# al8n/serf

Measured on NVIDIA H100. Metric: gossip edge-updates/sec @10M nodes, higher is better.
Workload: dtype u32

## Files before the change

### serf_b200/csrc/serfsim.cu

```cuda
#include <algorithm>
#include <cmath>
#include <cstdio>
#include <cstdlib>
#include <cstring>
#include <string>
#include <unordered_set>
#include <vector>

#include "../../include/serfsim.h"
#include "tick_kernel.cuh"
#include "wire.cuh"

using namespace sfs;

namespace {

thread_local std::string g_err;

int fail(int code, const std::string& msg) { g_err = msg; return code; }

#define CU(call)                                                                              \
  do {                                                                                        \
    cudaError_t e_ = (call);                                                                  \
    if (e_ != cudaSuccess)                                                                    \
// ... 50 lines not shown
    tab.push_back((u32)ticks);
  }
  return tab;
}

struct Switches {
  int gridmul = 2;
  bool minb5 = false;
  bool tma = false;
  bool tma_sync = false;
  bool udeg = true;
  u32 ahead = 1;
  u32 sv = 1;
  bool compact = true;
  bool dedup = true;
  bool no_skip = false;
  bool no_jump = false;
  u32 chunk = 0;
  double win_factor = 1.25;
  bool no_fuse = false;
  int l2_persist = 0;
  bool l2_window = false;
  bool verbose = false;
  bool debug_loop = false;
  bool xtiming = false;
};

Switches read_switches() {
  auto num = [](const char* name, int dflt) { const char* e = getenv(name); return e ? atoi(e) : dflt; };
  auto set = [](const char* name) { return getenv(name) != nullptr; };
  Switches s;
  s.gridmul = num("SERFSIM_GRIDMUL", s.gridmul); if (s.gridmul < 1) s.gridmul = 2;
  s.minb5 = num("SERFSIM_MINB", 0) == 5;
  s.tma = num("SERFSIM_TMA", s.tma) != 0;
  s.tma_sync = num("SERFSIM_TMA_SYNC", s.tma_sync) != 0;
  s.udeg = num("SERFSIM_UDEG", s.udeg) != 0;
  s.ahead = (u32)std::min(2, std::max(0, num("SERFSIM_AHEAD", s.ahead)));
  s.sv = (u32)std::min(2, std::max(0, num("SERFSIM_SV", s.sv)));
  s.compact = num("SERFSIM_COMPACT", s.compact) != 0;
  s.dedup = num("SERFSIM_DEDUP", s.dedup) != 0;
  s.no_skip = num("SERFSIM_NO_SKIP", s.no_skip) != 0;
  s.no_jump = set("SERFSIM_NO_JUMP");
  s.chunk = set("SERFSIM_CHUNK") ? (u32)std::max(1, num("SERFSIM_CHUNK", 1)) : 0u;
  if (const char* e = getenv("SERFSIM_WIN_FACTOR")) s.win_factor = atof(e);
  s.no_fuse = set("SERFSIM_NO_FUSE");
  s.l2_persist = num("SERFSIM_L2_PERSIST", s.l2_persist);
  s.l2_window = num("SERFSIM_L2_WINDOW", s.l2_window) != 0;
  s.verbose = set("SERFSIM_VERBOSE");
  s.debug_loop = set("SERFSIM_DEBUG_LOOP");
  s.xtiming = set("SERFSIM_XTIMING");
  return s;
}

}

// ... 15 lines not shown
  const u64** d_peer_snap_node = nullptr;
  u8* d_hot[2] = {nullptr, nullptr};
  u8* d_hot_static = nullptr;
  u32* d_node_due = nullptr;
  u32* d_carry = nullptr;
  u32* d_tile_due = nullptr;
  u32* d_sched = nullptr;
  u32 n_tiles = 0;
  u32* d_rowptr = nullptr;
  u32* d_col = nullptr;
  u32 *d_ev_node = nullptr, *d_ev_op = nullptr, *d_ev_slot = nullptr;
  size_t ev_cap = 0;
  u64* d_trace = nullptr;
  u32* d_kinds = nullptr;
  u32* d_view_kinds = nullptr;
  u32 trace_cap = 0;
  u32* d_overflow = nullptr;
  u32* pin_overflow = nullptr;
  u32* d_subj = nullptr;
  u64* d_scratch = nullptr;
  void* d_stage = nullptr;
  UeTable ue_table{};
  uint4* d_ue_state = nullptr;
  u32* d_ue_inbox[2] = {nullptr, nullptr};
  u32* d_ue_ltime = nullptr;
  wire::UeWire ue_wire{};
  u8* d_ue_entries = nullptr;
  u64* d_ue_totals = nullptr;
  u32 ue_injected = 0;
  uint4* d_ue_snap = nullptr;
// ... 62 lines not shown
  std::vector<cudaEvent_t> tick_ev;
  std::vector<cudaEvent_t> mid_ev;
};

namespace {

int slot_of(const serfsim* h, u32 node) {
  for (u32 s = 0; s < h->R; ++s) if (h->subj[s] == node) return (int)s;
  return -1;
}

int ensure_trace(serfsim* h, u32 need) {
  if (need <= h->trace_cap) return 0;
  u32 cap = std::max<u32>(1024, h->trace_cap);
  while (cap < need) cap *= 2;
  u64* nt = nullptr; u32* nk = nullptr; u32* nv = nullptr; u64* ng = nullptr;
  const bool sharded = h->cfg.world_size > 1;
  CU(cudaMalloc(&nt, (size_t)cap * 8 * sizeof(u64)));
  CU(cudaMalloc(&nk, ((size_t)cap + 1) * 4 * sizeof(u32)));
  CU(cudaMalloc(&nv, ((size_t)cap + 1) * h->R * 4 * sizeof(u32)));
  CU(cudaMemsetAsync(nt, 0, (size_t)cap * 8 * sizeof(u64), h->stream));
  CU(cudaMemsetAsync(nk, 0, ((size_t)cap + 1) * 4 * sizeof(u32), h->stream));
  CU(cudaMemsetAsync(nv, 0, ((size_t)cap + 1) * h->R * 4 * sizeof(u32), h->stream));
  if (sharded) { CU(cudaMalloc(&ng, (size_t)cap * 8 * sizeof(u64))); CU(cudaMemsetAsync(ng, 0, (size_t)cap * 8 * sizeof(u64), h->stream)); }
  if (h->d_trace) {
    CU(cudaMemcpyAsync(nt, h->d_trace, (size_t)h->trace_cap * 8 * sizeof(u64), cudaMemcpyDeviceToDevice, h->stream));
    CU(cudaMemcpyAsync(nk, h->d_kinds, ((size_t)h->trace_cap + 1) * 4 * sizeof(u32), cudaMemcpyDeviceToDevice, h->stream));
    CU(cudaMemcpyAsync(nv, h->d_view_kinds, ((size_t)h->trace_cap + 1) * h->R * 4 * sizeof(u32), cudaMemcpyDeviceToDevice, h->stream));
    if (sharded) CU(cudaMemcpyAsync(ng, h->d_grow, (size_t)h->trace_cap * 8 * sizeof(u64), cudaMemcpyDeviceToDevice, h->stream));
    CU(cudaStreamSynchronize(h->stream));
    cudaFree(h->d_trace); cudaFree(h->d_kinds); cudaFree(h->d_view_kinds); cudaFree(h->d_grow);
  }
  h->d_trace = nt; h->d_kinds = nk; h->d_view_kinds = nv; h->d_grow = ng; h->trace_cap = cap;
  return 0;
}

int upload_ops(serfsim* h) {
  if (!h->ops_dirty) return 0;
  std::stable_sort(h->ops.begin(), h->ops.end(), [](const HostOp& a, const HostOp& b) { return a.tick != b.tick ? a.tick < b.tick : a.seq < b.seq; });
  const size_t n = h->ops.size();
  if (n > h->ev_cap) {
    size_t cap = std::max<size_t>(1024, h->ev_cap);
    while (cap < n) cap *= 2;
    if (h->d_ev_node) { cudaFree(h->d_ev_node); cudaFree(h->d_ev_op); cudaFree(h->d_ev_slot); }
    CU(cudaMalloc(&h->d_ev_node, cap * 4)); CU(cudaMalloc(&h->d_ev_op, cap * 4)); CU(cudaMalloc(&h->d_ev_slot, cap * 4));
    h->ev_cap = cap;
  }
  if (n) {
// ... 32 lines not shown
    if (__builtin_popcount(h->ever_down) != 1) return TickRun::General;
    return h->sw.sv == 2 ? TickRun::Check : TickRun::Dual;
  }
  if (ops_at(h, t) || reap_tick(h, t) || t + 1 >= CARRY_TICKS) return TickRun::General;
  return h->sw.sv == 2 ? TickRun::Check : TickRun::Passes;
}
bool view_kinds_valid(const serfsim* h, u32 t) {
  return tick_run(h, t) == TickRun::Passes && !pp_tick(h, t);
}

TickParams at_view(const serfsim* h, const TickParams& p, u32 s) {
  TickParams q = p;
  q.sv_wshift = s;
  q.rec = p.rec + 2 * (size_t)s * h->stride; q.qword = p.qword + (size_t)s * h->stride;
  q.inbox_rd = p.inbox_rd + (size_t)s * h->stride; q.inbox_wr = p.inbox_wr + (size_t)s * h->stride;
  q.subj[0] = p.subj[s]; q.down_mask = (p.down_mask >> s) & 1u;
  q.tiles_per_cta = (h->n_tiles + h->grid_sv - 1) / h->grid_sv;
  return q;
}

int grow_events(std::vector<cudaEvent_t>& ev, size_t n) {
  while (ev.size() < n) { cudaEvent_t e; CU(cudaEventCreate(&e)); ev.push_back(e); }
  return 0;
}

int ue_cluster_ltimes(serfsim* h, u32 lt[MAX_UEVENTS]) {
  CU(cudaMemcpy(lt, h->d_ue_ltime, MAX_UEVENTS * sizeof(u32), cudaMemcpyDeviceToHost));
  if (h->cfg.world_size > 1 && h->allreduce) {
    u64 v[MAX_UEVENTS];
    for (u32 e = 0; e < MAX_UEVENTS; ++e) v[e] = (((h->ue_injected >> e) & 1u) && h->ue_origin[e] - h->first < h->count) ? lt[e] : 0;
// ... 26 lines not shown
  p.rec = h->d_rec; p.qword = h->d_qword; p.inbox_rd = h->d_inbox[(t & 1) ^ 1]; p.inbox_wr = h->d_inbox[t & 1];
  p.node_state = h->d_node; p.busy = h->d_busy; p.watch = h->d_watch; p.row_ptr = h->d_rowptr; p.col = h->d_col;
  p.ev_node = h->d_ev_node; p.ev_op = h->d_ev_op; p.ev_slot = h->d_ev_slot;
  p.row = h->d_trace + (size_t)t * 8;
  p.kinds_prev = h->d_kinds + (size_t)t * 4;
  p.kinds_cur = h->d_kinds + ((size_t)t + 1) * 4;
  p.overflow = h->d_overflow;
  p.hot_rd = h->d_hot[(t & 1) ^ 1]; p.hot_wr = h->d_hot[t & 1];
  p.stage_col_bytes = h->stage_col_bytes;
  p.reap_now = reap_tick(h, t) ? 1u : 0u;
  p.tombstone_ticks = h->cfg.tombstone_timeout_ticks; p.reconnect_ticks = h->cfg.reconnect_timeout_ticks; p.intent_ticks = h->cfg.recent_intent_timeout_ticks;
  p.stride = h->stride; p.n_tiles = h->n_tiles; p.tiles_per_cta = (h->n_tiles + h->grid - 1) / h->grid;
  p.force_all = (h->cfg.trace != 0) || h->sw.no_skip || p.reap_now;
  p.compact = h->sw.compact ? 1u : 0u;
  p.dedup = h->sw.dedup ? 1u : 0u;
  p.udeg = h->udeg; p.ahead = h->sw.ahead;
  p.tile_due = h->d_tile_due; p.node_due = h->d_node_due; p.hot_static = h->d_hot_static; p.sched = h->d_sched;
  p.sleep_on = (h->sw.no_skip || h->byz_on) ? 0u : 1u;
  p.pp_every = (u32)std::max(0, h->cfg.push_pull_interval_ticks); p.reap_every = h->cfg.reap_interval_ticks;
  p.host_idle_until = h->d_pin_ctl + 2;
  const bool sharded = h->cfg.world_size > 1;
  const u32 xpar = h->xepoch & 1;
  p.world = (u32)h->cfg.world_size; p.rank = (u32)h->cfg.rank; p.shard_size = h->shard_size; p.win_cap = h->win_cap;
  p.win_data = h->d_peer_data[xpar]; p.send_count = h->d_send_count;
  p.peer_ctrl = h->d_peer_ctrl; p.stamp = h->xepoch + 1; p.xpar = xpar; p.loopback = h->loopback ? 1u : 0u;
  p.fuse_publish = (sharded && !h->byz_on && !h->sw.no_fuse) ? 1u : 0u;
  p.shard_inv = (u32)(0x100000000ull / h->shard_size); p.xcap = p.world > 1 ? 392u / (p.world - 1) : 0u;
  if (h->gate_on) {
    const u64* grow = sharded ? h->d_grow : h->d_trace;
    Gate& g = p.gate;
// ... 251 lines not shown
  CU(cudaMemsetAsync(h->d_ue_ltime, 0, MAX_UEVENTS * 4, h->stream));
  CU(cudaMemsetAsync(h->d_ue_totals, 0, 8 * 8, h->stream));
  CU(cudaGetLastError());
  return 0;
}

int do_reset(serfsim* h, u64 seed) {
  h->cfg.seed = seed; h->tick = 0; h->ops.clear(); h->op_keys.clear(); h->ops_dirty = false; h->rows.clear();
  h->up_mask = (h->R >= 32) ? 0xffffffffu : ((1u << h->R) - 1);
  h->ever_down = 0;
  h->reported.assign(h->R, (u8)ST_ALIVE);
  const size_t inbox_bytes = (size_t)3 * h->R * h->stride * sizeof(u32);
  launch_init_state(h->d_rec, h->d_node, h->count, h->stride, h->R, h->cfg.init_status_ltime, h->cfg.init_clock, h->stream);
  CU(cudaMemsetAsync(h->d_inbox[0], 0, inbox_bytes, h->stream));
  CU(cudaMemsetAsync(h->d_inbox[1], 0, inbox_bytes, h->stream));
  CU(cudaStreamSynchronize(h->stream));
  *(volatile u32*)h->pin_overflow = 0;
  ((volatile u32*)h->pin_ctl)[2] = 0;
  CU(cudaMemsetAsync(h->d_busy, 0, h->stride, h->stream));
  CU(cudaMemsetAsync(h->d_qword, 0, (size_t)h->R * h->stride * 4, h->stream));
  CU(cudaMemsetAsync(h->d_hot[0], 0, h->n_tiles, h->stream));
  CU(cudaMemsetAsync(h->d_hot[1], 0, h->n_tiles, h->stream));
  CU(cudaMemsetAsync(h->d_tile_due, 0xff, (size_t)h->n_tiles * sizeof(u32), h->stream));
  CU(cudaMemsetAsync(h->d_node_due, 0xff, (size_t)h->stride * sizeof(u32), h->stream));
  if (h->d_carry) CU(cudaMemsetAsync(h->d_carry, 0, (size_t)h->stride * sizeof(u32), h->stream));
  CU(cudaMemsetAsync(h->d_sched, 0, SCHED_WORDS * sizeof(u32), h->stream));
  if (h->d_trace) {
    CU(cudaMemsetAsync(h->d_trace, 0, (size_t)h->trace_cap * 8 * sizeof(u64), h->stream));
    CU(cudaMemsetAsync(h->d_kinds, 0, ((size_t)h->trace_cap + 1) * 4 * sizeof(u32), h->stream));
    CU(cudaMemsetAsync(h->d_view_kinds, 0, ((size_t)h->trace_cap + 1) * h->R * 4 * sizeof(u32), h->stream));
  }
  if (h->d_grow) CU(cudaMemsetAsync(h->d_grow, 0, (size_t)h->trace_cap * 8 * sizeof(u64), h->stream));
  CU(cudaMemsetAsync(h->d_runctl, 0, 2 * sizeof(u32), h->stream));
  if (h->d_send_count) CU(cudaMemsetAsync(h->d_send_count, 0, sizeof(u32) * 8, h->stream));
  { int rc = ue_reset(h); if (rc) return rc; }
  if (h->d_anomaly) { CU(cudaMemsetAsync(h->d_anomaly, 0, h->stride, h->stream)); CU(cudaMemsetAsync(h->d_byz_totals, 0, 4 * 8, h->stream)); }
  { int rc = refresh_watchers(h); if (rc) return rc; }
  CU(cudaStreamSynchronize(h->stream));
  return 0;
}

void free_all(serfsim* h) {
  for (void* p : h->ipc_opened) cudaIpcCloseMemHandle(p);
  for (cudaEvent_t e : h->tick_ev) cudaEventDestroy(e);
  cudaFree(h->d_hot_static); cudaFree(h->d_tile_due); cudaFree(h->d_node_due); cudaFree(h->d_carry); cudaFree(h->d_sched);
  cudaFree(h->d_hot[0]); cudaFree(h->d_hot[1]); cudaFree(h->d_busy); cudaFree(h->d_watch); cudaFree(h->d_snap_rec); cudaFree(h->d_snap_node); cudaFree(h->d_peer_snap_rec); cudaFree(h->d_peer_snap_node);
  cudaFree(h->d_qword);
  cudaFree(h->d_rec); cudaFree(h->d_inbox[0]); cudaFree(h->d_inbox[1]); cudaFree(h->d_node); cudaFree(h->d_rowptr); cudaFree(h->d_col);
  cudaFree(h->d_ev_node); cudaFree(h->d_ev_op); cudaFree(h->d_ev_slot); cudaFree(h->d_trace); cudaFree(h->d_kinds); cudaFree(h->d_view_kinds);
  if (h->pin_overflow) cudaFreeHost(h->pin_overflow);
  cudaFree(h->d_subj); cudaFree(h->d_scratch); cudaFree(h->d_stage);
  cudaFree(h->d_byz_ids); cudaFree(h->d_anomaly); cudaFree(h->d_byz_totals); cudaFree(h->d_peer_anomaly);
  cudaFree(h->d_ue_snap); cudaFree(h->d_peer_ue_snap);
  cudaFree(h->d_ue_entries);
  cudaFree(h->d_ue_state); cudaFree(h->d_ue_inbox[0]); cudaFree(h->d_ue_inbox[1]); cudaFree(h->d_ue_ltime); cudaFree(h->d_ue_totals);
  for (int par = 0; par < 2; ++par) { cudaFree(h->d_win_data[par]); cudaFree(h->d_peer_data[par]); }
  cudaFree(h->d_ctrl); cudaFree(h->d_send_count); cudaFree(h->d_peer_ctrl);
  for (auto& b : h->res) { cudaFree(b.d); if (b.copied) cudaEventDestroy(b.copied); }
  if (h->ev_extracted) cudaEventDestroy(h->ev_extracted);
  if (h->copy_stream) cudaStreamDestroy(h->copy_stream);
  if (h->pin_ctl) cudaFreeHost(h->pin_ctl);
  cudaFree(h->d_runctl); cudaFree(h->d_grow);
  if (h->ev0) cudaEventDestroy(h->ev0);
  if (h->ev1) cudaEventDestroy(h->ev1);
// ... 121 lines not shown
  CUB(cudaMalloc(&h->d_hot_static, h->n_tiles)); CUB(cudaMalloc(&h->d_tile_due, (size_t)h->n_tiles * sizeof(u32))); CUB(cudaMalloc(&h->d_node_due, (size_t)h->stride * sizeof(u32))); CUB(cudaMalloc(&h->d_sched, SCHED_WORDS * sizeof(u32)));
  CUB(cudaMemset(h->d_hot_static, 0, h->n_tiles));
  if (h->R > 1 && cfg->world_size <= 1) CUB(cudaMalloc(&h->d_carry, (size_t)h->stride * sizeof(u32)));
  CUB(cudaHostAlloc(&h->pin_overflow, sizeof(u32), cudaHostAllocMapped));
  CUB(cudaHostGetDevicePointer(&h->d_overflow, h->pin_overflow, 0));
  *h->pin_overflow = 0;
  CUB(cudaMalloc(&h->d_subj, MAX_SLOTS * 4)); CUB(cudaMalloc(&h->d_scratch, 64 * 8));
  CUB(cudaMalloc(&h->d_stage, (size_t)h->count * 8));
  CUB(cudaMalloc(&h->d_runctl, 2 * sizeof(u32)));
  CUB(cudaMemset(h->d_runctl, 0, 2 * sizeof(u32)));
  CUB(cudaHostAlloc(&h->pin_ctl, 4 * sizeof(u32), cudaHostAllocMapped));
  CUB(cudaHostGetDevicePointer(&h->d_pin_ctl, h->pin_ctl, 0));
  h->pin_ctl[0] = h->pin_ctl[1] = h->pin_ctl[2] = h->pin_ctl[3] = 0;
  CUB(cudaMemcpy(h->d_subj, h->subj.data(), h->R * 4, cudaMemcpyHostToDevice));
  h->sw = read_switches();
  cudaDeviceGetAttribute(&h->sms, cudaDevAttrMultiProcessorCount, dev);
  if (h->sms <= 0) h->sms = 132;
  const int ctas_r1 = cfg->world_size > 1 ? tick_ctas_per_sm_r1s() : tick_ctas_per_sm_r1();
  h->ctas_per_sm = h->R > 1 ? tick_ctas_per_sm_rn() : h->sw.minb5 ? 5 : ctas_r1;
  h->grid = tick_grid_size(h->count, h->ctas_per_sm, h->sms, h->sw.gridmul);
  h->grid_sv = tick_grid_size(h->count, ctas_r1, h->sms, h->sw.gridmul);
  {
    int max_persist = 0, max_window = 0;
    cudaDeviceGetAttribute(&max_persist, cudaDevAttrMaxPersistingL2CacheSize, dev);
    cudaDeviceGetAttribute(&max_window, cudaDevAttrMaxAccessPolicyWindowSize, dev);
    h->l2_persist_max = (size_t)max_persist; h->l2_window_max = (size_t)max_window;
    if (h->sw.l2_persist && max_persist > 0) cudaDeviceSetLimit(cudaLimitPersistingL2CacheSize, (size_t)max_persist);
    if (h->sw.verbose) fprintf(stderr, "serfsim: L2 persisting max %d B, window max %d B, persist %d window %d\n", max_persist, max_window, h->sw.l2_persist, (int)h->sw.l2_window);
  }
  if (cfg->world_size > 1) {
// ... 654 lines not shown
```

### serf_b200/csrc/tick_kernel.cu

```cuda
#include <cstdlib>

#include "tick_kernel.cuh"
#include "byz.cuh"

namespace sfs {

namespace {

constexpr int BLOCK = 256;
#ifndef SFS_MB_R1
#define SFS_MB_R1 3
#endif
#ifndef SFS_MB_R1S
#define SFS_MB_R1S SFS_MB_R1
#endif
#ifndef SFS_MB_RN
#define SFS_MB_RN 1
#endif
constexpr u32 TILE_SHIFT = 8;
constexpr u32 MAX_TILES_PER_CTA = 1024;
static_assert((1u << TILE_SHIFT) == BLOCK, "tile = block");

struct Words { u32 w[8]; };

// ... 20 lines not shown
__device__ __forceinline__ u32 ld_u32_stream(const u32* ptr, u64 pol) {
  u32 v; asm volatile("ld.global.L1::no_allocate.L2::cache_hint.u32 %0, [%1], %2;" : "=r"(v) : "l"(ptr), "l"(pol)); return v;
}
__device__ __forceinline__ void st_u32_stream(u32* ptr, u32 v, u64 pol) {
  asm volatile("st.global.L2::cache_hint.u32 [%0], %1, %2;" :: "l"(ptr), "r"(v), "l"(pol) : "memory");
}
__device__ __forceinline__ void st_u64_stream(u64* ptr, u64 v, u64 pol) {
  asm volatile("st.global.L2::cache_hint.u64 [%0], %1, %2;" :: "l"(ptr), "l"(v), "l"(pol) : "memory");
}
__device__ __forceinline__ void red_max_resident(u32* ptr, u32 v, u64 pol) {
  asm volatile("red.relaxed.gpu.global.max.L2::cache_hint.u32 [%0], %1, %2;" :: "l"(ptr), "r"(v), "l"(pol) : "memory");
}
__device__ __forceinline__ u32 peek_inbox(const u32* ptr, u64 pol) {
  u32 v; asm volatile("ld.global.L1::no_allocate.L2::cache_hint.u32 %0, [%1], %2;" : "=r"(v) : "l"(ptr), "l"(pol)); return v;
}
__device__ __forceinline__ void st_release_sys(u32* ptr, u32 v) { asm volatile("st.release.sys.global.u32 [%0], %1;" :: "l"(ptr), "r"(v) : "memory"); }
__device__ __forceinline__ u32 ld_acquire_sys(const u32* ptr) { u32 f; asm volatile("ld.acquire.sys.global.u32 %0, [%1];" : "=r"(f) : "l"(ptr) : "memory"); return f; }
#else
inline u64 policy_evict_first() { return 0; }
inline u64 policy_evict_last() { return 0; }
inline Words ld_rec256(const uint4* ptr, u64) { emu::probes[8] += 32; Words r; const u32* q = reinterpret_cast<const u32*>(ptr); for (int i = 0; i < 8; ++i) r.w[i] = q[i]; return r; }
inline void st_rec256(uint4* ptr, const Words& r, u64) { emu::probes[9] += 32; u32* q = reinterpret_cast<u32*>(ptr); for (int i = 0; i < 8; ++i) q[i] = r.w[i]; }
inline u64 ld_u64_stream(const u64* ptr, u64) { emu::probes[10] += 8; return *ptr; }
inline u32 ld_u32_stream(const u32* ptr, u64) { emu::probes[11] += 4; return *ptr; }
inline void st_u32_stream(u32* ptr, u32 v, u64) { emu::probes[12] += 4; *ptr = v; }
inline void st_u64_stream(u64* ptr, u64 v, u64) { emu::probes[13] += 8; *ptr = v; }
inline void red_max_resident(u32* ptr, u32 v, u64) { emu::probes[14] += 4; if (v > *ptr) *ptr = v; }
inline u32 peek_inbox(const u32* ptr, u64) { emu::probes[11] += 4; return *ptr; }
inline void st_release_sys(u32* ptr, u32 v) { __atomic_store_n(ptr, v, __ATOMIC_RELEASE); }
inline u32 ld_acquire_sys(const u32* ptr) {
  static thread_local const u32* last = nullptr;
  static thread_local unsigned long spins = 0;
  if (ptr != last) { last = ptr; spins = 0; }
  if (++spins > 64) emu::polite_wait(spins);
  return __atomic_load_n(ptr, __ATOMIC_ACQUIRE);
}
#endif

#ifndef SERFSIM_EMU
__device__ __forceinline__ u32 smem_u32(const void* p) { return (u32)__cvta_generic_to_shared(p); }
__device__ __forceinline__ void mbar_init(u64* bar, u32 count) { asm volatile("mbarrier.init.shared::cta.b64 [%0], %1;" :: "r"(smem_u32(bar)), "r"(count) : "memory"); }
__device__ __forceinline__ void mbar_arrive_expect_tx(u64* bar, u32 bytes) {
  asm volatile("mbarrier.arrive.expect_tx.shared::cta.b64 _, [%0], %1;" :: "r"(smem_u32(bar)), "r"(bytes) : "memory");
// ... 71 lines not shown
    const u32 pos = base + (u32)__popc(peers & ((1u << lane) - 1u));
#else
    const u32 wid = threadIdx.x >> 5;
    const u32 pos = atomicAdd(&xs->cnt[wid][shard], 1u);
#endif
    if (pos < xcap(p)) {
      xs->buf[wid * XW_TOTAL + xseg(p, shard) + pos] = e;
    } else {
      const u32 g = atomicAdd(p.send_count + shard, 1u);
      if (g < p.win_cap) p.win_data[shard][(size_t)p.rank * p.win_cap + g] = e;
      else *p.overflow = 2;
    }
  }
}

template <int FMAX>
__device__ __forceinline__ void send_deduped(const TickParams& p, u32* plane, const u32 (&tg)[FMAX], u32 n, u32 val1, u64 pol_last, bool mark) {
  u32 held[FMAX];
#pragma unroll
  for (int k = 0; k < FMAX; ++k) held[k] = ((u32)k < n && p.dedup) ? peek_inbox(plane + (tg[k] - p.first), pol_last) : 0u;
#pragma unroll
  for (int k = 0; k < FMAX; ++k)
    if ((u32)k < n) deliver<false>(p, nullptr, plane, tg[k], 0, 0, val1, pol_last, mark, held[k]);
}

constexpr u32 XW_RESERVE_MAX = 128;
__device__ __forceinline__ bool flush_xwarp(const TickParams& p, XStage* xs, bool force, u32& resv, u32& rlen) {
  const u32 lane = threadIdx.x & 31, wid = threadIdx.x >> 5;
  __syncwarp();
  bool wrote = false;
  u32 want = 0;
  const u32 mine = lane < p.world ? xs->cnt[wid][lane] : 0u;
// ... 99 lines not shown

struct Pre { u32 busy, mL, mJ, mM, any, qw, mailmask, qmask, keep, nd; };
__device__ __forceinline__ u32 carry_of(const TickParams& p, u32 vl) {
  const u32 w = p.carry[vl];
  return (w >> 8) == ((p.tick + 1u) & (CARRY_TICKS - 1u)) ? (w & 0xffu) : 0u;
}
template <bool R1, bool PASS = false>
__device__ __forceinline__ Pre prefetch_node(const TickParams& p, u32 vl, bool kL, bool kJ, bool kM, u64 pol_first, bool due, u32 keep = 0) {
  const u32 nl = p.stride, R = p.R, s_hi = R1 ? 1u : R;
  Pre x;
  x.busy = p.busy[vl];
  x.nd = (!R1 && due) ? p.node_due[vl] : NO_DEADLINE;
  x.keep = R1 ? 0u : keep;
  x.mL = x.mJ = x.mM = x.qw = 0; x.any = 0; x.mailmask = 0; x.qmask = 0;
  for (u32 s2 = 0; s2 < s_hi; ++s2) {
    const u32 l = kL ? ld_u32_stream(p.inbox_rd + (size_t)(KIND_LEAVE * R + s2) * nl + vl, pol_first) : 0u;
    const u32 j = kJ ? ld_u32_stream(p.inbox_rd + (size_t)(KIND_JOIN * R + s2) * nl + vl, pol_first) : 0u;
    const u32 m = kM ? ld_u32_stream(p.inbox_rd + (size_t)(KIND_ML * R + s2) * nl + vl, pol_first) : 0u;
    const u32 q = p.qword[(size_t)s2 * nl + vl];
    SFS_COUNT(6, 4);
    if (R1 || s2 == x.keep) { x.mL = l; x.mJ = j; x.mM = m; x.qw = q; }
    x.any |= l | j | m;
    x.mailmask |= ((l | j | m) ? 1u : 0u) << s2;
    x.qmask |= (q ? 1u : 0u) << s2;
  }
  if (PASS) x.any |= x.qw | ((due && (carry_of(p, vl) & CARRY_TDUE)) ? 1u : 0u);
  return x;
}
template <bool PASS = false>
__device__ __forceinline__ u32 busy_business(u32 busy) { return busy & (PASS ? 6u : 7u); }
template <bool PASS = false>
__device__ __forceinline__ bool node_active(const TickParams& p, const Pre& x, bool due) {
  return busy_business<PASS>(x.busy) != 0 || x.any != 0 || p.reap_now != 0 || (due && (x.busy & 8u) && x.nd <= p.tick);
// ... 154 lines not shown
  bool awake = false, has_timer = false, dl_moved = false;

  const u32 all_views = (R >= 32u) ? 0xffffffffu : ((1u << R) - 1u);
  const bool visit_all = R1 || TRACE || p.reap_now || (busy & 2u) || timers_due || !p.sleep_on;
  u32 todo = visit_all ? all_views : ((pre.mailmask | pre.qmask | (p.probe_every ? (SFS_WMASK() & p.down_mask) : 0u)) & all_views);
  if (!R1) SFS_COUNT(5, R - (u32)__popc(todo));

  Words nxt = {};
  u32 nL = 0, nJ = 0, nM = 0, nq = 0;
  auto load_view = [&](u32 s2, Words& w, u32& q, u32& iL, u32& iJ, u32& iM) {
    const size_t idn = (size_t)s2 * nl + vl;
    w = ld_rec256(p.rec + 2 * idn, pol_first);
    if (s2 == pre.keep) { q = pre.qw; iL = pre.mL; iJ = pre.mJ; iM = pre.mM; return; }
    q = p.qword[idn];
    SFS_COUNT(6, 4);
    iL = kL ? ld_u32_stream(p.inbox_rd + (size_t)(KIND_LEAVE * R + s2) * nl + vl, pol_first) : 0;
    iJ = kJ ? ld_u32_stream(p.inbox_rd + (size_t)(KIND_JOIN * R + s2) * nl + vl, pol_first) : 0;
    iM = kM ? ld_u32_stream(p.inbox_rd + (size_t)(KIND_ML * R + s2) * nl + vl, pol_first) : 0;
  };
#ifndef SFS_VIEW_PREFETCH
#define SFS_VIEW_PREFETCH 0
#endif
  u32 s = R;
  if (R1) { s = 0; todo = 0; }
  else if (todo) {
    s = (u32)__ffs((int)todo) - 1u; todo &= todo - 1u;
    u32 q0;
    if (ahead && s == pre.keep) { cur = ah.rec; q0 = pre.qw; mL = pre.mL; mJ = pre.mJ; mM = pre.mM; SFS_PROBE(18); }
    else load_view(s, cur, q0, mL, mJ, mM);
    merge_q(cur, q0);
    first_view = s;
  }
#pragma unroll 1
// ... 39 lines not shown
        if (!have_targets) {
          if (ahead) nt = pick_finish<FMAX>(v, ah.cand, tg);
          else {
            u32 cand[FMAX];
            pick_issue<FMAX, STAGED>(p, sv, v, row0, deg, pol_first, cand);
            nt = pick_finish<FMAX>(v, cand, tg);
          }
          have_targets = true;
        }
        u32* const planeL = p.inbox_wr + (size_t)(KIND_LEAVE * R + s) * nl;
        u32* const planeJ = p.inbox_wr + (size_t)(KIND_JOIN * R + s) * nl;
        u32* const planeM = p.inbox_wr + (size_t)(KIND_ML * R + s) * nl;
        const u32 vL = leave_key(r.qleave, (r.flags & FLAG_QPRUNE) != 0) + 1, vJ = r.qjoin + 1, vM = ml_key(r) + 1;
        const u32 sL = min(r.txl, nt), sJ = min(r.txj, nt), sM = min(r.txm, nt);
        if (!SHARDED) {
          send_deduped<FMAX>(p, planeL, tg, sL, vL, pol_last, mark);
          send_deduped<FMAX>(p, planeJ, tg, sJ, vJ, pol_last, mark);
          send_deduped<FMAX>(p, planeM, tg, sM, vM, pol_last, mark);
        } else {
#pragma unroll
          for (int k = 0; k < FMAX; ++k) {
            if ((u32)k < sL) deliver<SHARDED>(p, xs, planeL, tg[k], KIND_LEAVE, s, vL, pol_last, mark);
            if ((u32)k < sJ) deliver<SHARDED>(p, xs, planeJ, tg[k], KIND_JOIN, s, vJ, pol_last, mark);
            if ((u32)k < sM) deliver<SHARDED>(p, xs, planeM, tg[k], KIND_ML, s, vM, pol_last, mark);
          }
        }
        if (R1) { c.kLJ += sL | (sJ << 16); c.kM += sM; c.pe += min(mx, nt) << 16; }
        else { c.kL += sL; c.kJ += sJ; c.kM += sM; c.edges += min(mx, nt); }
        max_tx = max(max_tx, mx);
        r.txl -= sL; r.txj -= sJ; r.txm -= sM;
      }
      if (self && sstate == SS_LEAVING && r.txl == 0 && r.mlstate == ML_ALIVE) {
        r.mlstate = ML_LEFT; r.qfrom = 0; r.txm = limit; sstate = SS_LEFT;
// ... 168 lines not shown
      sched[SCHED_LOCAL_QUIET] = quiet ? 1u : 0u; sched[SCHED_LOCAL_UNTIL] = until;
    }
    const u32 awake_n = sched[SCHED_AWAKE];
    sched[SCHED_AWAKE] = 0; sched[SCHED_UE_ACTIVITY] = 0; sched[SCHED_TICKET] = 0;
    const u32 sv_next = (p.sv_mode == SV_SINGLE && (row[2] != 0 || awake_n != 0)) ? (1u << p.sv_slot) : 0u;
    const u32 sv_base = p.tick >= sched[SCHED_VIEWS_FROM] ? sched[SCHED_VIEWS_NEW] : sched[SCHED_VIEWS_OLD];
    sched[SCHED_VIEWS_OLD] = sv_base; sched[SCHED_VIEWS_NEW] = sched[SCHED_VIEWS_NEXT] | sv_next; sched[SCHED_VIEWS_FROM] = p.tick + 1; sched[SCHED_VIEWS_NEXT] = 0;
  }
  if (p.world > 1 && p.fuse_publish) {
    __syncthreads();
    __threadfence();
    publish_to_peer(threadIdx.x, p.world, p.rank, p.xpar, p.stamp, p.loopback, p.peer_ctrl, p.send_count, row, sched);
  }
}

template <bool TRACE, int FMAX, bool SHARDED, bool R1, int MB, bool PASS = false>
__global__ void __launch_bounds__(BLOCK, MB) tick_kernel(const __grid_constant__ TickParams p) {
  __shared__ u8 hot_s[MAX_TILES_PER_CTA];
  __shared__ u64 red[8][BLOCK / 32];
  __shared__ int dsusp_s;
  __shared__ __align__(16) unsigned char xs_mem[SHARDED ? sizeof(XStage) : 16];
  XStage* xs = reinterpret_cast<XStage*>(xs_mem);
  if (gate_closed(p.gate, blockIdx.x == 0 && threadIdx.x == 0)) return;
  if (tick_is_idle(p.sched, p.tick, p.ev_begin, p.ev_end)) { if (PASS ? p.sv_slot == 0 : p.sv_mode != SV_SINGLE) write_idle_row<TRACE>(p); return; }
  u32 sv_views = 0xffffffffu;
  bool work = true, carry_out = false;
  if (PASS) {
    const u32 sv_base = p.tick >= p.sched[SCHED_VIEWS_FROM] ? p.sched[SCHED_VIEWS_NEW] : p.sched[SCHED_VIEWS_OLD];
    const u32 views = (sv_base | p.views_host) & ((1u << p.sv_R) - 1u);
    work = (views >> p.sv_slot) & 1u;
    carry_out = (views >> p.sv_slot) > 1u;
    if (work) SFS_PROBE(21);
    else if (p.sv_slot != 0 && p.sv_slot + 1u < p.sv_R) return;
  } else if (p.sv_mode != SV_OFF) {
    const u32 sv_base = p.tick >= p.sched[SCHED_VIEWS_FROM] ? p.sched[SCHED_VIEWS_NEW] : p.sched[SCHED_VIEWS_OLD];
    const u32 views = (sv_base | p.views_host) & ((1u << p.sv_R) - 1u);
    const bool single = views == (1u << p.sv_slot);
    if (p.sv_mode == SV_SINGLE) { if (!single) return; SFS_PROBE(21); }
    else if (p.sv_mode == SV_GENERAL && single) return;
    if (p.sv_mode == SV_CHECK && (single || p.world == 1)) sv_views = views;
  }
  if (threadIdx.x == 0) dsusp_s = 0;
  Counters c = {};
  const u32* const kv = PASS ? p.view_kinds_prev : p.kinds_prev;
  const bool kL = kv[KIND_LEAVE] != 0, kJ = kv[KIND_JOIN] != 0, kM = kv[KIND_ML] != 0;
  const u64 pol_first = policy_evict_first(), pol_last = policy_evict_last();
  const int lane = threadIdx.x & 31;
  if (SHARDED && threadIdx.x < (BLOCK / 32) * MAX_WORLD) xs->cnt[threadIdx.x / MAX_WORLD][threadIdx.x % MAX_WORLD] = 0;
  bool wrote_remote = false;
  u32 resv = 0, rlen = 0;

  const u32 prev_msgs = p.kinds_prev[KIND_LEAVE] + p.kinds_prev[KIND_JOIN] + p.kinds_prev[KIND_ML];
  const bool dense_now = prev_msgs >= (p.n_tiles >> 1) + 1;
  const bool all_hot = p.force_all || p.kinds_prev[3] != 0;
  const bool mark = !dense_now;
  const u32 own_msgs = PASS ? kv[KIND_LEAVE] + kv[KIND_JOIN] + kv[KIND_ML] : prev_msgs;
  const bool saturated = own_msgs >= (p.n_local >> 1);
// ... 121 lines not shown
    bool pend = false;
    u32 mind = NO_DEADLINE;
    int dsusp = 0;
    if (vl < p.n_local) pend = process_node<TRACE, FMAX, SHARDED, R1, false, PASS>(p, StageView{}, xs, vl, pre, kL, kJ, kM, mark, saturated, (hot_s[i] & 2u) != 0, pol_first, pol_last, c, mind, dsusp, ah, first_view, sv_views, carry_out);
    if (mark && __any_sync(0xffffffffu, pend) && lane == 0) p.hot_wr[tile0 + i] = 1;
    note_timers(p, tile0 + i, mind, dsusp, &dsusp_s);
    if (SHARDED) wrote_remote |= flush_xwarp(p, xs, false, resv, rlen);
    i = j;
  }
  }
  if (SHARDED) {
    wrote_remote |= flush_xwarp(p, xs, true, resv, rlen);
    if (wrote_remote) __threadfence_system();
  }
  __syncthreads();
  finish_tick<TRACE, R1, PASS>(p, c, red, dsusp_s);
}

#ifndef SERFSIM_EMU
template <bool TRACE, int FMAX, bool SHARDED, bool BARSYNC>
__global__ void __launch_bounds__(BLOCK, 3) tick_kernel_tma(const __grid_constant__ TickParams p) {
  extern __shared__ __align__(128) unsigned char stage_mem[];
  __shared__ u8 hot_s[MAX_TILES_PER_CTA];
  __shared__ u16 hot_list[MAX_TILES_PER_CTA];
  __shared__ u32 n_hot_s;
  __shared__ u64 red[8][BLOCK / 32];
  __shared__ __align__(8) u64 full_bar[2], empty_bar[2];
  __shared__ u32 col_base_s[2], col_ok_s[2];
  __shared__ int dsusp_s;
  if (gate_closed(p.gate, blockIdx.x == 0 && threadIdx.x == 0)) return;
// ... 526 lines not shown
```

### serf_b200/csrc/tick_kernel.cuh

```cuda
#pragma once
#include <cuda_runtime.h>

#include "record.cuh"
#include "uevent.cuh"

#if defined(SERFSIM_EMU) && defined(__CUDACC__)
#error "SERFSIM_EMU is the host-only test build of tests/emu (g++); the product is built by nvcc without it"
#endif
#ifndef SERFSIM_EMU
#define SFS_LAUNCH(grid, block, smem, stream, ...) __VA_ARGS__<<<(grid), (block), (smem), (stream)>>>
constexpr int SFS_SMS = 132;
#else
constexpr int SFS_SMS = 1;
#endif
#ifdef SERFSIM_EMU
#define SFS_PROBE(i) (emu::probes[i]++)
#define SFS_COUNT(i, n) (emu::probes[i] += (n))
#else
#define SFS_PROBE(i) ((void)0)
#define SFS_COUNT(i, n) ((void)0)
#endif

namespace sfs {

// ... 61 lines not shown
  u32 udeg;
  u32* tile_due;
  u32* node_due;
  const u8* hot_static;
  u32* sched;
  u32 sleep_on;
  u32 pp_every, reap_every;
  u32* const* peer_ctrl; u32 stamp, xpar, loopback, fuse_publish;
  u32 shard_inv, xcap;
  u32 sv_wshift;
  u32 sv_mode, views_host, sv_slot, sv_R;
  u32 ahead;
  u32* host_idle_until;
  u32* carry;
  const u32* view_kinds_prev; u32* view_kinds_cur;
};
constexpr u32 SCHED_TICKET = 0, SCHED_IDLE_UNTIL = 1, SCHED_UE_ACTIVITY = 2, SCHED_AWAKE = 3, SCHED_SUSPECTS = 4 ,
              SCHED_LOCAL_QUIET = 6, SCHED_LOCAL_UNTIL = 7 ,
              SCHED_VIEWS_NEW = 8 , SCHED_VIEWS_NEXT = 9 ,
              SCHED_VIEWS_OLD = 10 , SCHED_VIEWS_FROM = 11, SCHED_WORDS = 12;
constexpr u32 SV_OFF = 0, SV_GENERAL = 1, SV_SINGLE = 2, SV_CHECK = 3, SV_PASS = 4;
constexpr u32 CARRY_PK = 0xfu, CARRY_AWAKE = 0x10u, CARRY_TDUE = 0x20u, CARRY_SEEN = 0x40u, CARRY_TICKS = 1u << 24;
constexpr u32 NO_DEADLINE = 0xffffffffu;
__device__ __forceinline__ bool tick_is_idle(const u32* sched, u32 tick, u32 ev_begin, u32 ev_end) {
  return sched && ev_begin == ev_end && tick < sched[SCHED_IDLE_UNTIL];
}

constexpr u32 CTRL_U32 = 2 * 16;
constexpr u32 CTRL_SUMS_OFF = CTRL_U32 * 4;
constexpr u32 CTRL_FIELDS = 11;
// ... 104 lines not shown
```

Before: 21.78 billion.

## Add wave bitmap inbox encoding for gossip messages matching the current max value

```diff
diff --git a/serf_b200/csrc/serfsim.cu b/serf_b200/csrc/serfsim.cu
--- a/serf_b200/csrc/serfsim.cu
+++ b/serf_b200/csrc/serfsim.cu
@@ -88,6 +88,7 @@
   u32 sv = 1;
   bool compact = true;
   bool dedup = true;
+  bool wave = true;
   bool no_skip = false;
   bool no_jump = false;
   u32 chunk = 0;
@@ -113,6 +114,7 @@
   s.sv = (u32)std::min(2, std::max(0, num("SERFSIM_SV", s.sv)));
   s.compact = num("SERFSIM_COMPACT", s.compact) != 0;
   s.dedup = num("SERFSIM_DEDUP", s.dedup) != 0;
+  s.wave = num("SERFSIM_WAVE", s.wave) != 0;
   s.no_skip = num("SERFSIM_NO_SKIP", s.no_skip) != 0;
   s.no_jump = set("SERFSIM_NO_JUMP");
   s.chunk = set("SERFSIM_CHUNK") ? (u32)std::max(1, num("SERFSIM_CHUNK", 1)) : 0u;
@@ -158,6 +160,8 @@
   u64* d_trace = nullptr;
   u32* d_kinds = nullptr;
   u32* d_view_kinds = nullptr;
+  u32* d_wave = nullptr;
+  u32* d_wbits[2] = {nullptr, nullptr};
   u32 trace_cap = 0;
   u32* d_overflow = nullptr;
   u32* pin_overflow = nullptr;
@@ -250,7 +254,7 @@
   if (need <= h->trace_cap) return 0;
   u32 cap = std::max<u32>(1024, h->trace_cap);
   while (cap < need) cap *= 2;
-  u64* nt = nullptr; u32* nk = nullptr; u32* nv = nullptr; u64* ng = nullptr;
+  u64* nt = nullptr; u32* nk = nullptr; u32* nv = nullptr; u32* nw = nullptr; u64* ng = nullptr;
   const bool sharded = h->cfg.world_size > 1;
   CU(cudaMalloc(&nt, (size_t)cap * 8 * sizeof(u64)));
   CU(cudaMalloc(&nk, ((size_t)cap + 1) * 4 * sizeof(u32)));
@@ -258,16 +262,18 @@
   CU(cudaMemsetAsync(nt, 0, (size_t)cap * 8 * sizeof(u64), h->stream));
   CU(cudaMemsetAsync(nk, 0, ((size_t)cap + 1) * 4 * sizeof(u32), h->stream));
   CU(cudaMemsetAsync(nv, 0, ((size_t)cap + 1) * h->R * 4 * sizeof(u32), h->stream));
+  if (h->d_wbits[0]) { CU(cudaMalloc(&nw, ((size_t)cap + 1) * h->R * 4 * sizeof(u32))); CU(cudaMemsetAsync(nw, 0, ((size_t)cap + 1) * h->R * 4 * sizeof(u32), h->stream)); }
   if (sharded) { CU(cudaMalloc(&ng, (size_t)cap * 8 * sizeof(u64))); CU(cudaMemsetAsync(ng, 0, (size_t)cap * 8 * sizeof(u64), h->stream)); }
   if (h->d_trace) {
     CU(cudaMemcpyAsync(nt, h->d_trace, (size_t)h->trace_cap * 8 * sizeof(u64), cudaMemcpyDeviceToDevice, h->stream));
     CU(cudaMemcpyAsync(nk, h->d_kinds, ((size_t)h->trace_cap + 1) * 4 * sizeof(u32), cudaMemcpyDeviceToDevice, h->stream));
     CU(cudaMemcpyAsync(nv, h->d_view_kinds, ((size_t)h->trace_cap + 1) * h->R * 4 * sizeof(u32), cudaMemcpyDeviceToDevice, h->stream));
+    if (nw) CU(cudaMemcpyAsync(nw, h->d_wave, ((size_t)h->trace_cap + 1) * h->R * 4 * sizeof(u32), cudaMemcpyDeviceToDevice, h->stream));
     if (sharded) CU(cudaMemcpyAsync(ng, h->d_grow, (size_t)h->trace_cap * 8 * sizeof(u64), cudaMemcpyDeviceToDevice, h->stream));
     CU(cudaStreamSynchronize(h->stream));
-    cudaFree(h->d_trace); cudaFree(h->d_kinds); cudaFree(h->d_view_kinds); cudaFree(h->d_grow);
-  }
-  h->d_trace = nt; h->d_kinds = nk; h->d_view_kinds = nv; h->d_grow = ng; h->trace_cap = cap;
+    cudaFree(h->d_trace); cudaFree(h->d_kinds); cudaFree(h->d_view_kinds); cudaFree(h->d_wave); cudaFree(h->d_grow);
+  }
+  h->d_trace = nt; h->d_kinds = nk; h->d_view_kinds = nv; h->d_wave = nw; h->d_grow = ng; h->trace_cap = cap;
   return 0;
 }
 
@@ -330,6 +336,10 @@
   q.sv_wshift = s;
   q.rec = p.rec + 2 * (size_t)s * h->stride; q.qword = p.qword + (size_t)s * h->stride;
   q.inbox_rd = p.inbox_rd + (size_t)s * h->stride; q.inbox_wr = p.inbox_wr + (size_t)s * h->stride;
+  if (p.wbits_rd) {
+    q.wbits_rd = p.wbits_rd + (size_t)s * (h->stride / 32); q.wbits_wr = p.wbits_wr + (size_t)s * (h->stride / 32);
+    q.wave_rd = p.wave_rd + 4 * s; q.wave_snd = p.wave_snd + 4 * s; q.wave_cur = p.wave_cur + 4 * s;
+  }
   q.subj[0] = p.subj[s]; q.down_mask = (p.down_mask >> s) & 1u;
   q.tiles_per_cta = (h->n_tiles + h->grid_sv - 1) / h->grid_sv;
   return q;
@@ -386,6 +396,10 @@
   p.force_all = (h->cfg.trace != 0) || h->sw.no_skip || p.reap_now;
   p.compact = h->sw.compact ? 1u : 0u;
   p.dedup = h->sw.dedup ? 1u : 0u;
+  if (h->d_wbits[0] && !h->stage_col_bytes) {
+    p.wbits_rd = h->d_wbits[(t & 1) ^ 1]; p.wbits_wr = h->d_wbits[t & 1];
+    p.wave_rd = h->d_wave + (size_t)(t ? t - 1 : 0) * h->R * 4; p.wave_snd = h->d_wave + (size_t)t * h->R * 4; p.wave_cur = h->d_wave + ((size_t)t + 1) * h->R * 4;
+  }
   p.udeg = h->udeg; p.ahead = h->sw.ahead;
   p.tile_due = h->d_tile_due; p.node_due = h->d_node_due; p.hot_static = h->d_hot_static; p.sched = h->d_sched;
   p.sleep_on = (h->sw.no_skip || h->byz_on) ? 0u : 1u;
@@ -667,6 +681,7 @@
   launch_init_state(h->d_rec, h->d_node, h->count, h->stride, h->R, h->cfg.init_status_ltime, h->cfg.init_clock, h->stream);
   CU(cudaMemsetAsync(h->d_inbox[0], 0, inbox_bytes, h->stream));
   CU(cudaMemsetAsync(h->d_inbox[1], 0, inbox_bytes, h->stream));
+  for (u32* b : h->d_wbits) if (b) CU(cudaMemsetAsync(b, 0, inbox_bytes / 32, h->stream));
   CU(cudaStreamSynchronize(h->stream));
   *(volatile u32*)h->pin_overflow = 0;
   ((volatile u32*)h->pin_ctl)[2] = 0;
@@ -682,6 +697,7 @@
     CU(cudaMemsetAsync(h->d_trace, 0, (size_t)h->trace_cap * 8 * sizeof(u64), h->stream));
     CU(cudaMemsetAsync(h->d_kinds, 0, ((size_t)h->trace_cap + 1) * 4 * sizeof(u32), h->stream));
     CU(cudaMemsetAsync(h->d_view_kinds, 0, ((size_t)h->trace_cap + 1) * h->R * 4 * sizeof(u32), h->stream));
+    if (h->d_wave) CU(cudaMemsetAsync(h->d_wave, 0, ((size_t)h->trace_cap + 1) * h->R * 4 * sizeof(u32), h->stream));
   }
   if (h->d_grow) CU(cudaMemsetAsync(h->d_grow, 0, (size_t)h->trace_cap * 8 * sizeof(u64), h->stream));
   CU(cudaMemsetAsync(h->d_runctl, 0, 2 * sizeof(u32), h->stream));
@@ -701,6 +717,7 @@
   cudaFree(h->d_qword);
   cudaFree(h->d_rec); cudaFree(h->d_inbox[0]); cudaFree(h->d_inbox[1]); cudaFree(h->d_node); cudaFree(h->d_rowptr); cudaFree(h->d_col);
   cudaFree(h->d_ev_node); cudaFree(h->d_ev_op); cudaFree(h->d_ev_slot); cudaFree(h->d_trace); cudaFree(h->d_kinds); cudaFree(h->d_view_kinds);
+  cudaFree(h->d_wave); cudaFree(h->d_wbits[0]); cudaFree(h->d_wbits[1]);
   if (h->pin_overflow) cudaFreeHost(h->pin_overflow);
   cudaFree(h->d_subj); cudaFree(h->d_scratch); cudaFree(h->d_stage);
   cudaFree(h->d_byz_ids); cudaFree(h->d_anomaly); cudaFree(h->d_byz_totals); cudaFree(h->d_peer_anomaly);
@@ -852,6 +869,7 @@
   h->pin_ctl[0] = h->pin_ctl[1] = h->pin_ctl[2] = h->pin_ctl[3] = 0;
   CUB(cudaMemcpy(h->d_subj, h->subj.data(), h->R * 4, cudaMemcpyHostToDevice));
   h->sw = read_switches();
+  if (h->sw.wave && cfg->world_size <= 1) { CUB(cudaMalloc(&h->d_wbits[0], inbox_bytes / 32)); CUB(cudaMalloc(&h->d_wbits[1], inbox_bytes / 32)); }
   cudaDeviceGetAttribute(&h->sms, cudaDevAttrMultiProcessorCount, dev);
   if (h->sms <= 0) h->sms = 132;
   const int ctas_r1 = cfg->world_size > 1 ? tick_ctas_per_sm_r1s() : tick_ctas_per_sm_r1();
diff --git a/serf_b200/csrc/tick_kernel.cu b/serf_b200/csrc/tick_kernel.cu
--- a/serf_b200/csrc/tick_kernel.cu
+++ b/serf_b200/csrc/tick_kernel.cu
@@ -58,6 +58,9 @@
 __device__ __forceinline__ u32 peek_inbox(const u32* ptr, u64 pol) {
   u32 v; asm volatile("ld.global.L1::no_allocate.L2::cache_hint.u32 %0, [%1], %2;" : "=r"(v) : "l"(ptr), "l"(pol)); return v;
 }
+__device__ __forceinline__ void red_or_resident(u32* ptr, u32 v, u64 pol) {
+  asm volatile("red.relaxed.gpu.global.or.L2::cache_hint.b32 [%0], %1, %2;" :: "l"(ptr), "r"(v), "l"(pol) : "memory");
+}
 __device__ __forceinline__ void st_release_sys(u32* ptr, u32 v) { asm volatile("st.release.sys.global.u32 [%0], %1;" :: "l"(ptr), "r"(v) : "memory"); }
 __device__ __forceinline__ u32 ld_acquire_sys(const u32* ptr) { u32 f; asm volatile("ld.acquire.sys.global.u32 %0, [%1];" : "=r"(f) : "l"(ptr) : "memory"); return f; }
 #else
@@ -71,6 +74,7 @@
 inline void st_u64_stream(u64* ptr, u64 v, u64) { emu::probes[13] += 8; *ptr = v; }
 inline void red_max_resident(u32* ptr, u32 v, u64) { emu::probes[14] += 4; if (v > *ptr) *ptr = v; }
 inline u32 peek_inbox(const u32* ptr, u64) { emu::probes[11] += 4; return *ptr; }
+inline void red_or_resident(u32* ptr, u32 v, u64) { emu::probes[14] += 4; *ptr |= v; }
 inline void st_release_sys(u32* ptr, u32 v) { __atomic_store_n(ptr, v, __ATOMIC_RELEASE); }
 inline u32 ld_acquire_sys(const u32* ptr) {
   static thread_local const u32* last = nullptr;
@@ -172,8 +176,34 @@
   }
 }
 
+__device__ __forceinline__ u32* wave_plane(u32* base, u32 kind, u32 s, u32 R, u32 nl) { return base ? base + (size_t)(kind * R + s) * (nl >> 5) : nullptr; }
+__shared__ u32 wave_s[MAX_SLOTS * 4];
+__device__ __forceinline__ u32 wave_mail(const TickParams& p, u32 word, u32 kind, u32 s2, u32 vl, u64 pol) {
+  if (!p.wbits_rd) return word;
+  const u32 b = peek_inbox(wave_plane(p.wbits_rd, kind, s2, p.R, p.stride) + (vl >> 5), pol);
+  return ((b >> (vl & 31)) & 1u) ? max(word, p.wave_rd[4 * s2 + kind]) : word;
+}
+
 template <int FMAX>
-__device__ __forceinline__ void send_deduped(const TickParams& p, u32* plane, const u32 (&tg)[FMAX], u32 n, u32 val1, u64 pol_last, bool mark) {
+__device__ __forceinline__ void send_deduped(const TickParams& p, u32* plane, u32* bits, u32 wave, u32* wmax, const u32 (&tg)[FMAX], u32 n, u32 val1, u64 pol_last, bool mark) {
+  if (bits && n) {
+    if (val1 > *wmax) atomicMax(wmax, val1);
+    if (val1 == wave) {
+      u32 held[FMAX];
+#pragma unroll
+      for (int k = 0; k < FMAX; ++k) held[k] = ((u32)k < n && p.dedup) ? peek_inbox(bits + ((tg[k] - p.first) >> 5), pol_last) : 0u;
+#pragma unroll
+      for (int k = 0; k < FMAX; ++k)
+        if ((u32)k < n) {
+          const u32 dl = tg[k] - p.first, bit = 1u << (dl & 31);
+          if (!(held[k] & bit)) { red_or_resident(bits + (dl >> 5), bit, pol_last); SFS_PROBE(29); }
+          else SFS_PROBE(30);
+          if (mark) p.hot_wr[dl >> TILE_SHIFT] = 1;
+        }
+      return;
+    }
+    SFS_PROBE(31);
+  }
   u32 held[FMAX];
 #pragma unroll
   for (int k = 0; k < FMAX; ++k) held[k] = ((u32)k < n && p.dedup) ? peek_inbox(plane + (tg[k] - p.first), pol_last) : 0u;
@@ -303,9 +333,9 @@
   x.keep = R1 ? 0u : keep;
   x.mL = x.mJ = x.mM = x.qw = 0; x.any = 0; x.mailmask = 0; x.qmask = 0;
   for (u32 s2 = 0; s2 < s_hi; ++s2) {
-    const u32 l = kL ? ld_u32_stream(p.inbox_rd + (size_t)(KIND_LEAVE * R + s2) * nl + vl, pol_first) : 0u;
-    const u32 j = kJ ? ld_u32_stream(p.inbox_rd + (size_t)(KIND_JOIN * R + s2) * nl + vl, pol_first) : 0u;
-    const u32 m = kM ? ld_u32_stream(p.inbox_rd + (size_t)(KIND_ML * R + s2) * nl + vl, pol_first) : 0u;
+    const u32 l = kL ? wave_mail(p, ld_u32_stream(p.inbox_rd + (size_t)(KIND_LEAVE * R + s2) * nl + vl, pol_first), KIND_LEAVE, s2, vl, pol_first) : 0u;
+    const u32 j = kJ ? wave_mail(p, ld_u32_stream(p.inbox_rd + (size_t)(KIND_JOIN * R + s2) * nl + vl, pol_first), KIND_JOIN, s2, vl, pol_first) : 0u;
+    const u32 m = kM ? wave_mail(p, ld_u32_stream(p.inbox_rd + (size_t)(KIND_ML * R + s2) * nl + vl, pol_first), KIND_ML, s2, vl, pol_first) : 0u;
     const u32 q = p.qword[(size_t)s2 * nl + vl];
     SFS_COUNT(6, 4);
     if (R1 || s2 == x.keep) { x.mL = l; x.mJ = j; x.mM = m; x.qw = q; }
@@ -490,9 +520,9 @@
     if (s2 == pre.keep) { q = pre.qw; iL = pre.mL; iJ = pre.mJ; iM = pre.mM; return; }
     q = p.qword[idn];
     SFS_COUNT(6, 4);
-    iL = kL ? ld_u32_stream(p.inbox_rd + (size_t)(KIND_LEAVE * R + s2) * nl + vl, pol_first) : 0;
-    iJ = kJ ? ld_u32_stream(p.inbox_rd + (size_t)(KIND_JOIN * R + s2) * nl + vl, pol_first) : 0;
-    iM = kM ? ld_u32_stream(p.inbox_rd + (size_t)(KIND_ML * R + s2) * nl + vl, pol_first) : 0;
+    iL = kL ? wave_mail(p, ld_u32_stream(p.inbox_rd + (size_t)(KIND_LEAVE * R + s2) * nl + vl, pol_first), KIND_LEAVE, s2, vl, pol_first) : 0;
+    iJ = kJ ? wave_mail(p, ld_u32_stream(p.inbox_rd + (size_t)(KIND_JOIN * R + s2) * nl + vl, pol_first), KIND_JOIN, s2, vl, pol_first) : 0;
+    iM = kM ? wave_mail(p, ld_u32_stream(p.inbox_rd + (size_t)(KIND_ML * R + s2) * nl + vl, pol_first), KIND_ML, s2, vl, pol_first) : 0;
   };
 #ifndef SFS_VIEW_PREFETCH
 #define SFS_VIEW_PREFETCH 0
@@ -562,9 +592,10 @@
         const u32 vL = leave_key(r.qleave, (r.flags & FLAG_QPRUNE) != 0) + 1, vJ = r.qjoin + 1, vM = ml_key(r) + 1;
         const u32 sL = min(r.txl, nt), sJ = min(r.txj, nt), sM = min(r.txm, nt);
         if (!SHARDED) {
-          send_deduped<FMAX>(p, planeL, tg, sL, vL, pol_last, mark);
-          send_deduped<FMAX>(p, planeJ, tg, sJ, vJ, pol_last, mark);
-          send_deduped<FMAX>(p, planeM, tg, sM, vM, pol_last, mark);
+          const bool wave = p.wbits_wr != nullptr;
+          send_deduped<FMAX>(p, planeL, wave_plane(p.wbits_wr, KIND_LEAVE, s, R, nl), wave ? p.wave_snd[4 * s + KIND_LEAVE] : 0u, wave_s + 4 * s + KIND_LEAVE, tg, sL, vL, pol_last, mark);
+          send_deduped<FMAX>(p, planeJ, wave_plane(p.wbits_wr, KIND_JOIN, s, R, nl), wave ? p.wave_snd[4 * s + KIND_JOIN] : 0u, wave_s + 4 * s + KIND_JOIN, tg, sJ, vJ, pol_last, mark);
+          send_deduped<FMAX>(p, planeM, wave_plane(p.wbits_wr, KIND_ML, s, R, nl), wave ? p.wave_snd[4 * s + KIND_ML] : 0u, wave_s + 4 * s + KIND_ML, tg, sM, vM, pol_last, mark);
         } else {
 #pragma unroll
           for (int k = 0; k < FMAX; ++k) {
@@ -763,6 +794,20 @@
   }
 }
 
+__device__ __forceinline__ void wave_end(const TickParams& p, const u8* hot_s, u32 tile0, u32 ntile, u32 views, bool kL, bool kJ, bool kM) {
+  constexpr u32 WPT = (1u << TILE_SHIFT) >> 5;
+  const u32 kinds = (kL ? 1u << KIND_LEAVE : 0u) | (kJ ? 1u << KIND_JOIN : 0u) | (kM ? 1u << KIND_ML : 0u);
+  if (kinds)
+    for (u32 i = threadIdx.x; i < ntile * WPT; i += BLOCK) {
+      if (!(hot_s[i / WPT] & 1u)) continue;
+      const u32 w = tile0 * WPT + i;
+      for (u32 s2 = 0; s2 < views; ++s2)
+        for (u32 k = 0; k < 3; ++k)
+          if ((kinds >> k) & 1u) wave_plane(p.wbits_rd, k, s2, p.R, p.stride)[w] = 0u;
+    }
+  if (threadIdx.x < views * 4 && wave_s[threadIdx.x]) atomicMax(p.wave_cur + threadIdx.x, wave_s[threadIdx.x]);
+}
+
 template <bool TRACE, int FMAX, bool SHARDED, bool R1, int MB, bool PASS = false>
 __global__ void __launch_bounds__(BLOCK, MB) tick_kernel(const __grid_constant__ TickParams p) {
   __shared__ u8 hot_s[MAX_TILES_PER_CTA];
@@ -790,6 +835,7 @@
     if (p.sv_mode == SV_CHECK && (single || p.world == 1)) sv_views = views;
   }
   if (threadIdx.x == 0) dsusp_s = 0;
+  if (!SHARDED && threadIdx.x < MAX_SLOTS * 4) wave_s[threadIdx.x] = 0;
   Counters c = {};
   const u32* const kv = PASS ? p.view_kinds_prev : p.kinds_prev;
   const bool kL = kv[KIND_LEAVE] != 0, kJ = kv[KIND_JOIN] != 0, kM = kv[KIND_ML] != 0;
@@ -941,6 +987,7 @@
     if (wrote_remote) __threadfence_system();
   }
   __syncthreads();
+  if (!SHARDED && p.wbits_wr) wave_end(p, hot_s, tile0, ntile, R1 ? 1u : p.R, kL, kJ, kM);
   finish_tick<TRACE, R1, PASS>(p, c, red, dsusp_s);
 }
 
diff --git a/serf_b200/csrc/tick_kernel.cuh b/serf_b200/csrc/tick_kernel.cuh
--- a/serf_b200/csrc/tick_kernel.cuh
+++ b/serf_b200/csrc/tick_kernel.cuh
@@ -99,6 +99,10 @@
   u32* host_idle_until;
   u32* carry;
   const u32* view_kinds_prev; u32* view_kinds_cur;
+  u32* wbits_rd; u32* wbits_wr;
+  const u32* wave_rd;
+  const u32* wave_snd;
+  u32* wave_cur;
 };
 constexpr u32 SCHED_TICKET = 0, SCHED_IDLE_UNTIL = 1, SCHED_UE_ACTIVITY = 2, SCHED_AWAKE = 3, SCHED_SUSPECTS = 4 ,
               SCHED_LOCAL_QUIET = 6, SCHED_LOCAL_UNTIL = 7 ,
```

Result: faster. 27.15 billion (median of 6 runs) (+24.6%).
